# argmaxinc/WhisperKit

Hardware: AMD Instinct MI355X
Metric: audio-sec/sec (1/RTF), 30 s chunks: host PCM -> log-mel + encoder + greedy decode -> segments (higher is better)
Workload: dtype f16

## Files before the change

### whisperkit_amd/csrc/xabs.hip

```cpp
#include "dec_shared.h"
#include "knobs.h"

namespace wh {

typedef unsigned u32x4 __attribute__((ext_vector_type(4)));
typedef short s16x4 __attribute__((ext_vector_type(4)));
typedef f16 f16x2 __attribute__((ext_vector_type(2)));

__host__ __device__ __forceinline__ int xswz(int key) { return ((key & 3) << 2) | ((0x78 >> (2 * ((key >> 2) & 3))) & 3); }

__global__ void xabs_tile_wk_kernel(const f16* __restrict__ Wk, int d, int H, f16* __restrict__ out, size_t n_units) {
    const size_t o = (size_t)blockIdx.x * blockDim.x + threadIdx.x;
    if (o >= n_units) return;
    const int lane = (int)(o & 63);
    size_t t = o >> 6;
    const int kt = (int)(t & 3); t >>= 2;
    const int RT = d >> 5;
    const int rt = (int)(t % RT), h = (int)(t / RT);
    const int c = rt * 32 + (lane & 31), j0 = h * 64 + kt * 16 + 8 * (lane >> 5);
    f16x8 v;
#pragma unroll
    for (int i = 0; i < 8; ++i) v[i] = Wk[(size_t)(j0 + i) * d + c];
    *reinterpret_cast<f16x8*>(out + o * 8) = v;
}
void xabs_tile_wk(const f16* Wk, int d, int H, f16* out, hipStream_t st) {
    const size_t n_units = (size_t)H * (d / 32) * 4 * 64;
    xabs_tile_wk_kernel<<<(unsigned)((n_units + 255) / 256), 256, 0, st>>>(Wk, d, H, out, n_units);
}

template <int NHT, int WPB = 4>
__global__ __launch_bounds__(256, 2) void xabs_qk_kernel(const XabsArgs a) {
    const int tid = threadIdx.x, lane = tid & 63, wave = tid >> 6;
    const int h = blockIdx.y, bt = blockIdx.z;
    const int d = a.d, RT = d >> 5;
    const int j = lane & 31, hl = lane >> 5, gb = bt * 32 + j;
    f16x8 qh[4], ql[4];
    {
        const float* qp = a.q + (size_t)gb * d + h * 64 + hl * 8;
        float4 v0[4], v1[4];
#pragma unroll
        for (int kt = 0; kt < 4; ++kt) { v0[kt] = *reinterpret_cast<const float4*>(qp + kt * 16); v1[kt] = *reinterpret_cast<const float4*>(qp + kt * 16 + 4); }
#pragma unroll
        for (int kt = 0; kt < 4; ++kt) {
            const float z[8] = {v0[kt].x, v0[kt].y, v0[kt].z, v0[kt].w, v1[kt].x, v1[kt].y, v1[kt].z, v1[kt].w};
#pragma unroll
            for (int i = 0; i < 8; ++i) { f16 h_, l_; split_hilo(z[i], h_, l_); qh[kt][i] = h_; ql[kt][i] = l_; }
        }
    }
#pragma unroll
    for (int s = 0; s < 2; ++s) {
        const int rt = (blockIdx.x * WPB + wave) * 2 + s;
        const u32x4* wp = reinterpret_cast<const u32x4*>(a.wkT) + ((size_t)(h * RT + rt) * 4) * 64 + lane;
        u32x4 w[4];
#pragma unroll
        for (int kt = 0; kt < 4; ++kt) w[kt] = wp[kt * 64];
        f32x16 acc_h = {0}, acc_l = {0};
#pragma unroll
        for (int kt = 0; kt < 4; ++kt) {
            const f16x8 wf = __builtin_bit_cast(f16x8, w[kt]);
            acc_h = __builtin_amdgcn_mfma_f32_32x32x16_f16(wf, qh[kt], acc_h, 0, 0, 0);
            acc_l = __builtin_amdgcn_mfma_f32_32x32x16_f16(wf, ql[kt], acc_l, 0, 0, 0);
        }
        unsigned ph[4][2], pl[4][2];
#pragma unroll
        for (int g = 0; g < 4; ++g) {
            f16 zh[4], zl[4];
#pragma unroll
            for (int i = 0; i < 4; ++i) split_hilo(fmaf(acc_l[4 * g + i], 1.0f / 2048.0f, acc_h[4 * g + i]), zh[i], zl[i]);
            ph[g][0] = __builtin_bit_cast(unsigned, f16x2{zh[0], zh[1]});
            ph[g][1] = __builtin_bit_cast(unsigned, f16x2{zh[2], zh[3]});
            pl[g][0] = __builtin_bit_cast(unsigned, f16x2{zl[0], zl[1]});
            pl[g][1] = __builtin_bit_cast(unsigned, f16x2{zl[2], zl[3]});
        }
        u32x4 oh[2], ol[2];
#pragma unroll
        for (int u = 0; u < 2; ++u) {
#pragma unroll
            for (int i = 0; i < 2; ++i) {
                auto sh = __builtin_amdgcn_permlane32_swap(ph[u][i], ph[u + 2][i], false, false);
                auto sl = __builtin_amdgcn_permlane32_swap(pl[u][i], pl[u + 2][i], false, false);
                oh[u][i] = sh[0]; oh[u][2 + i] = sh[1];
                ol[u][i] = sl[0]; ol[u][2 + i] = sl[1];
            }
        }
        if (gb < a.batch) {
            const size_t o = ((size_t)gb * (NHT * 16) + h) * d + rt * 32 + 16 * hl;
            f16* lo_dst = h < 16 ? a.qf_lo + o : a.qf_hi + o + (size_t)8 * d;
#pragma unroll
            for (int u = 0; u < 2; ++u) {
                *reinterpret_cast<u32x4*>(a.qf_hi + o + 8 * u) = oh[u];
                *reinterpret_cast<u32x4*>(lo_dst + 8 * u) = ol[u];
            }
        }
    }
    if (a.gate && blockIdx.x == 0 && blockIdx.y == 0 && blockIdx.z == 0 && tid == 0) xattn_gate_acquire(a.gate);
}

template <int KSW, int NHT>
struct XabsQFrag { f16x8 h0[KSW], l0[KSW], p1[NHT == 2 ? KSW : 1]; };
template <int KSW, int NHT>
__device__ __forceinline__ void xabs_load_qfrag(const XabsArgs& a, int b, int c0, int lane, XabsQFrag<KSW, NHT>& q) {
    const int row = lane & 15, H = a.n_head, D = a.d;
    const size_t qo = ((size_t)b * (NHT * 16) + row) * D + c0 + (lane >> 4) * 8;
    const f16x8 zero = {0, 0, 0, 0, 0, 0, 0, 0};
    const bool real0 = row < H;
    const bool real1 = NHT == 2 && 16 + (row & 7) < H;
#pragma unroll
    for (int j = 0; j < KSW; ++j) {
        q.h0[j] = real0 ? *reinterpret_cast<const f16x8*>(a.qf_hi + qo + j * 32) : zero;
        q.l0[j] = real0 ? *reinterpret_cast<const f16x8*>(a.qf_lo + qo + j * 32) : zero;
        if constexpr (NHT == 2) q.p1[j] = real1 ? *reinterpret_cast<const f16x8*>(a.qf_hi + qo + (size_t)16 * D + j * 32) : zero;
    }
}
template <int KSW, int NHT>
__device__ __forceinline__ void xabs_s_tile(const f16x8 (&af)[KSW], const XabsQFrag<KSW, NHT>& q, int lane, float (&sreg)[NHT * 4]) {
    f32x4 sh = {0, 0, 0, 0}, sl = {0, 0, 0, 0}, sp = {0, 0, 0, 0};
#pragma unroll
    for (int j = 0; j < KSW; ++j) {
        sh = __builtin_amdgcn_mfma_f32_16x16x32_f16(af[j], q.h0[j], sh, 0, 0, 0);
        sl = __builtin_amdgcn_mfma_f32_16x16x32_f16(af[j], q.l0[j], sl, 0, 0, 0);
        if constexpr (NHT == 2) sp = __builtin_amdgcn_mfma_f32_16x16x32_f16(af[j], q.p1[j], sp, 0, 0, 0);
    }
#pragma unroll
    for (int r = 0; r < 4; ++r) sreg[r] = fmaf(sl[r], 1.0f / 2048.0f, sh[r]);
    if constexpr (NHT == 2) {
#pragma unroll
        for (int r = 0; r < 4; ++r) {
            const float lo = dpp_mov<kDppRor8>(sp[r]);
            sreg[4 + r] = (lane & 15) < 8 ? fmaf(lo, 1.0f / 2048.0f, sp[r]) : 0.0f;
        }
    }
}

constexpr int kXabsHalves = 7;
constexpr int kXabsSpStride = 32 * 17;
constexpr float kXabsDefer = 8.0f;
__host__ __device__ constexpr int xabs_lds_bytes_w(int nw, int ksw) { return kXabsHalves * 8 * nw * ksw * 64 + nw * kXabsSpStride * 4 + 1024 + 128; }
__host__ __device__ constexpr int xabs_lds_bytes(int cw) { return xabs_lds_bytes_w(8, cw); }

template <int KSW, int NHT, bool DBG, bool NTL, int NW = 8, bool MAP = false>
__global__ __launch_bounds__(NW * 64, 2) void xabs_attn_kernel(const XabsArgs a) {
    static_assert(NW == 8 || NW == 4, "the waves split the channels: 8, or 4 at d = 384");
    static_assert(4 * NW >= 16 * NHT, "4 softmax-owner heads per wave");
    constexpr int CW = KSW;
    constexpr int HWSH = NW == 8 ? 2 : 1, HW = NW / 2;
    constexpr int D = NW * KSW * 32, ROWB = D * 2, HALF = 8 * ROWB;
    static_assert(HALF == HW * CW * 1024, "a half tile is HW x CW pieces of 1 KB");
    extern __shared__ __attribute__((aligned(1024))) unsigned char smem[];
    float* spart = reinterpret_cast<float*>(smem + kXabsHalves * HALF);
    f16* pfrag = reinterpret_cast<f16*>(smem + kXabsHalves * HALF + NW * kXabsSpStride * 4);
    float* alpha_l = reinterpret_cast<float*>(smem + kXabsHalves * HALF + NW * kXabsSpStride * 4 + 1024);
    const int tid = threadIdx.x, lane = tid & 63;
    const int wave = __builtin_amdgcn_readfirstlane(tid >> 6);
    const int xr = blockIdx.x & 7, xq = blockIdx.x >> 3;
    const int S = a.n_split, H = a.n_head;
    const int spw = max(a.spw, 1), b1 = (a.batch + spw - 1) / spw;
    const int n_grp = (b1 + 3) >> 2, grp = (xq >> 2) * 8 + xr;
    const int sp = grp / n_grp, b_first = ((grp - sp * n_grp) << 2) + (xq & 3);
    if (a.gate && blockIdx.x == gridDim.x - 1 && tid == 0) xattn_gate_release(a.gate);
    if (sp >= S || b_first >= b1) return;
#define XPHASE(k) do { if constexpr (DBG) if (a.dbg && lane == 0 && (wave == 0 || wave == 5) && blockIdx.x < 64) \
        a.dbg[((blockIdx.x * 2 + (wave == 5)) * 2) * 16 + (k)] = __builtin_amdgcn_s_memtime(); } while (0)
    constexpr int NT = (kCtx + 15) / 16;
    const int tile_lo = sp * NT / S, tile_hi = (sp + 1) * NT / S, n = tile_hi - tile_lo;
  for (int b = b_first; b < a.batch; b += b1) {
    if (b != b_first) __syncthreads();
    XPHASE(9);
    int bc, bh = b;
    if constexpr (MAP) { bh = a.slot_home[b]; bc = bh; }
    else bc = a.cross_div > 1 ? b / a.cross_div : b;
    const unsigned char* enc = reinterpret_cast<const unsigned char*>(a.enc + (size_t)bc * kCtx * D);

    const int half_w = wave >> HWSH, wq = wave & (HW - 1);
    int p_off[CW];
#pragma unroll
    for (int p = 0; p < CW; ++p) {
        const int o = (wq * CW + p) * 1024 + lane * 16;
        const int row = o / ROWB, slot = (o - row * ROWB) >> 4;
        p_off[p] = (half_w * 8 + row) * ROWB + ((slot ^ xswz(half_w * 8 + row)) << 4);
    }
    int hi_mine = -1;
    auto issue = [&](int i) {
        unsigned char* dst = smem + ((2 * i + half_w) % kXabsHalves) * HALF + wq * (CW * 1024);
        const int t16 = (tile_lo + i) * 16;
#if defined(__HIP_DEVICE_COMPILE__)
        const __amdgpu_buffer_rsrc_t rs = __builtin_amdgcn_make_buffer_rsrc(const_cast<unsigned char*>(enc) + (size_t)t16 * ROWB, 0, (kCtx - t16) * ROWB, 0x00020000);
#pragma unroll
        for (int p = 0; p < CW; ++p)
            __builtin_amdgcn_raw_ptr_buffer_load_lds(rs, (__attribute__((address_space(3))) void*)(dst + p * 1024), 16, p_off[p], 0, 0, NTL ? 2 : 0);
#else
        (void)dst; (void)t16; (void)p_off;
#endif
        hi_mine = i;
    };
    auto wait_tile = [&](int k) {
        switch (hi_mine - k) {
            case 0: asm volatile("s_waitcnt vmcnt(0)" ::: "memory"); break;
            case 1: asm volatile("s_waitcnt vmcnt(%0)" ::"n"(CW) : "memory"); break;
            case 2: asm volatile("s_waitcnt vmcnt(%0)" ::"n"(2 * CW) : "memory"); break;
            default: asm volatile("s_waitcnt vmcnt(%0)" ::"n"(3 * CW) : "memory"); break;
        }
    };
    const SeqState* sq = a.seq + b;
    const int s_act = sq->active, s_done = sq->done, s_ti = sq->token_index;
    const int o_key = lane & 15, o_head = 4 * wave + (lane >> 4);
    const bool owner = o_head < 16 * NHT;
    int al_slot = -1;
    if (a.align && owner && o_head < H) al_slot = a.align_slot[a.layer * H + o_head];
    XabsQFrag<CW, NHT> qf;
    xabs_load_qfrag<CW, NHT>(a, b, wave * CW * 32, lane, qf);
    issue(0);
    if (n > 1) issue(1);
    if (n > 2) issue(2);
    if (n > 3 && half_w == 0) issue(3);
    if (tid < 32) alpha_l[tid] = 1.0f;
    if constexpr (NW == 8) pfrag[tid] = (f16)0.0f;
    else reinterpret_cast<unsigned*>(pfrag)[tid] = 0u;
    if (!(s_act && !s_done)) {
        asm volatile("s_waitcnt vmcnt(0)" ::: "memory");
        continue;
    }
    const int pos = min(max(s_ti, 0), kMaxTok - 1);
    float* raw = nullptr;
    if (al_slot >= 0 && pos + 1 < kMaxTok) raw = a.align + (((size_t)bh * kMaxTok + pos + 1) * a.n_align + al_slot) * kCtx;
    XPHASE(10);

    f32x16 acc[CW];
#pragma unroll
    for (int mt = 0; mt < CW; ++mt)
#pragma unroll
        for (int r = 0; r < 16; ++r) acc[mt][r] = 0.0f;
    float m_run = -INFINITY, l_run = 0.0f;
    const int s_key = lane & 15, s_kg = lane >> 4, s_sw = xswz(s_key);
    const int g16 = lane >> 4, sl = lane & 15;
    const int t_key0 = (g16 >> 1) * 8 + (sl >> 2), t_key1 = t_key0 + 4;
    const int t_c = (g16 & 1) * 2 + ((sl & 3) >> 1), t_b = (sl & 1) * 8;
    const int t_off0 = (t_key0 & 7) * ROWB + t_b, t_off1 = (t_key1 & 7) * ROWB + t_b, t_sw0 = xswz(t_key0), t_sw1 = xswz(t_key1);
    auto s_base = [&](int i) { return smem + ((2 * i + (s_key >> 3)) % kXabsHalves) * HALF + (s_key & 7) * ROWB; };
    auto t_base = [&](int i) { return smem + ((2 * i + (g16 >> 1)) % kXabsHalves) * HALF; };

    auto s_phase = [&](const unsigned char* row, float (&sreg)[NHT * 4]) {
        f16x8 af[CW];
#pragma unroll
        for (int j = 0; j < CW; ++j) {
            const int c = (wave * CW + j) * 4 + s_kg;
            af[j] = *reinterpret_cast<const f16x8*>(row + ((c ^ s_sw) << 4));
        }
        xabs_s_tile<CW, NHT>(af, qf, lane, sreg);
    };
    auto write_partials = [&](const float (&sreg)[NHT * 4]) {
        float* wpart = spart + wave * kXabsSpStride;
#pragma unroll
        for (int ht = 0; ht < NHT; ++ht)
#pragma unroll
            for (int r = 0; r < 4; ++r) wpart[(ht * 16 + (lane & 15)) * 17 + 4 * (lane >> 4) + r] = sreg[ht * 4 + r];
    };
    auto softmax = [&](int i) {
        float s = 0.0f;
#pragma unroll
        for (int v = 0; v < NW; ++v) s += spart[v * kXabsSpStride + o_head * 17 + o_key];
        const int t = (tile_lo + i) * 16 + o_key;
        const bool valid = t < kCtx;
        if (raw && valid) raw[t] = s;
        s = valid ? s : -INFINITY;
        float mt_ = s;
        mt_ = fmaxf(mt_, dpp_mov<kDppXor1>(mt_));
        mt_ = fmaxf(mt_, dpp_mov<kDppXor2>(mt_));
        mt_ = fmaxf(mt_, dpp_mov<kDppHalfMirror>(mt_));
        mt_ = fmaxf(mt_, dpp_mov<kDppMirror>(mt_));
        const float m_new = fmaxf(m_run, mt_);
        const float m_use = (m_new > m_run + kXabsDefer) ? m_new : m_run;
        const float al = __expf(m_run - m_use);
        float p = valid ? __expf(s - m_use) : 0.0f;
        if (o_head >= H) p = 0.0f;
        const f16 ph = (f16)p;
        float ps = (float)ph;
        ps += dpp_mov<kDppXor1>(ps);
        ps += dpp_mov<kDppXor2>(ps);
        ps += dpp_mov<kDppHalfMirror>(ps);
        ps += dpp_mov<kDppMirror>(ps);
        l_run = fmaf(l_run, al, ps);
        m_run = m_use;
        pfrag[(o_head | ((o_key >> 3) << 5)) * 8 + (o_key & 7)] = ph;
        if (o_key == 0) alpha_l[o_head] = (o_head < H) ? al : 1.0f;
    };
    auto pv = [&](const unsigned char* tile) {
        const f16x8 pf = *reinterpret_cast<const f16x8*>(pfrag + lane * 8);
        const float al = alpha_l[lane & 31];
        if (__builtin_amdgcn_ballot_w64(al != 1.0f)) {
#pragma unroll
            for (int mt = 0; mt < CW; ++mt)
#pragma unroll
                for (int r = 0; r < 16; ++r) acc[mt][r] *= al;
        }
#pragma unroll
        for (int mt = 0; mt < CW; ++mt) {
            const int c = (wave * CW + mt) * 4 + t_c;
            const s16x4 a0 = __builtin_amdgcn_ds_read_tr16_b64_v4i16((__attribute__((address_space(3))) s16x4*)(tile + t_off0 + ((c ^ t_sw0) << 4)));
            const s16x4 a1 = __builtin_amdgcn_ds_read_tr16_b64_v4i16((__attribute__((address_space(3))) s16x4*)(tile + t_off1 + ((c ^ t_sw1) << 4)));
            const f16x4 f0 = __builtin_bit_cast(f16x4, a0), f1 = __builtin_bit_cast(f16x4, a1);
            const f16x8 af = {f0[0], f0[1], f0[2], f0[3], f1[0], f1[1], f1[2], f1[3]};
            acc[mt] = __builtin_amdgcn_mfma_f32_32x32x16_f16(af, pf, acc[mt], 0, 0, 0);
        }
    };

    float sreg[NHT * 4];
    wait_tile(0);
    __syncthreads();
    s_phase(s_base(0), sreg);
    write_partials(sreg);
    if (n > 1) wait_tile(1);
    __syncthreads();
    XPHASE(11);
#define XSTAMP(k) do { if constexpr (DBG) if (a.dbg && (i == 10 || i == 11) && lane == 0 && (wave == 0 || wave == 5) && blockIdx.x < 64) \
        a.dbg[((blockIdx.x * 2 + (wave == 5)) * 2 + (i - 10)) * 16 + (k)] = __builtin_amdgcn_s_memtime(); } while (0)
    for (int i = 0; i < n; ++i) {
        XSTAMP(0);
        const bool work = !DBG || !(a.ablate & 2), fetch = !DBG || !(a.ablate & 1);
        if (work && i + 1 < n) s_phase(s_base(i + 1), sreg);
        XSTAMP(1);
        if (work && owner) softmax(i);
        XSTAMP(2);
        __syncthreads();
        XSTAMP(3);
        if (work && i + 1 < n) write_partials(sreg);
        XSTAMP(4);
        if (work) pv(t_base(i));
        XSTAMP(5);
        if (fetch && i + 2 < n) wait_tile(i + 2);
        XSTAMP(6);
        __syncthreads();
        XSTAMP(7);
        const int nx = i + 3 + (1 - half_w);
        if (fetch && nx < n) issue(nx);
        XSTAMP(8);
    }
#undef XSTAMP
    asm volatile("s_waitcnt vmcnt(0)" ::: "memory");
    XPHASE(12);
    if (owner && o_key == 0 && o_head < H) a.ml[((size_t)sp * H + o_head) * a.max_batch + b] = float2{m_run, l_run};
    {
        const int head = lane & 31, hl = lane >> 5;
        if (head < H) {
            float* pb = a.part + (((size_t)sp * H + head) * (D / 8)) * a.max_batch * 8 + (size_t)b * 8 + 4 * hl;
#pragma unroll
            for (int mt = 0; mt < CW; ++mt)
#pragma unroll
                for (int g = 0; g < 4; ++g) {
                    const int c8 = (wave * CW + mt) * 4 + g;
                    *reinterpret_cast<float4*>(pb + (size_t)c8 * a.max_batch * 8) = float4{acc[mt][4 * g], acc[mt][4 * g + 1], acc[mt][4 * g + 2], acc[mt][4 * g + 3]};
                }
        }
    }
    if constexpr (DBG) asm volatile("s_waitcnt vmcnt(0)" ::: "memory");
    XPHASE(13);
  }
#undef XPHASE
}


template <int S, int TW>
__global__ __launch_bounds__(256, 1) void xabs_vup_kernel(const XabsArgs a, int ks, int n_bt) {
    __shared__ float red[4][2][16][64];
    __shared__ int last_flag;
    const int tid = threadIdx.x, lane = tid & 63, wave = tid >> 6;
    const int d = a.d, H = a.n_head, KT = d >> 4;
    const int grp8 = blockIdx.x / (8 * n_bt), in8 = blockIdx.x % (8 * n_bt);
    const int xw = grp8 * 8 + (in8 & 7), bt = in8 >> 3;
    if (xw >= H * ks) return;
    const int h = xw % H, ksi = xw / H;
    const int kt0 = (ksi * 4 + wave) * TW;
    const int j = lane & 31, hl = lane >> 5;
    const int gbl = min(bt * 32 + j, a.max_batch - 1);
    float2 ml[S];
#pragma unroll
    for (int s = 0; s < S; ++s) ml[s] = a.ml[((size_t)s * H + h) * a.max_batch + gbl];
    const u32x4* wp = reinterpret_cast<const u32x4*>(a.wv_t) + ((size_t)(2 * h) * KT + kt0) * 64 + lane;
    const size_t sstride = (size_t)H * (d / 8) * a.max_batch * 8;
    const float* pp = a.part + ((size_t)h * (d / 8) + kt0 * 2 + hl) * a.max_batch * 8 + (size_t)gbl * 8;
    u32x4 w0[TW], w1[TW];
    f32x4 p0[TW][S], p1[TW][S];
#pragma unroll
    for (int i = 0; i < TW; ++i) { w0[i] = __builtin_nontemporal_load(wp + (size_t)i * 64); w1[i] = __builtin_nontemporal_load(wp + ((size_t)KT + i) * 64); }
#pragma unroll
    for (int i = 0; i < TW; ++i)
#pragma unroll
        for (int s = 0; s < S; ++s) {
            const float* q = pp + (size_t)s * sstride + (size_t)i * 2 * a.max_batch * 8;
            p0[i][s] = *reinterpret_cast<const f32x4*>(q);
            p1[i][s] = *reinterpret_cast<const f32x4*>(q + 4);
        }
#pragma unroll
    for (int i = 0; i < TW; ++i) {
        asm volatile("" : "+v"(w0[i]), "+v"(w1[i]));
#pragma unroll
        for (int s = 0; s < S; ++s) asm volatile("" : "+v"(p0[i][s]), "+v"(p1[i][s]));
    }
    float wn[S];
    {
        float mg = ml[0].x;
#pragma unroll
        for (int s = 1; s < S; ++s) mg = fmaxf(mg, ml[s].x);
        float lg = 0.0f;
#pragma unroll
        for (int s = 0; s < S; ++s) { wn[s] = __expf(ml[s].x - mg); lg = fmaf(wn[s], ml[s].y, lg); }
        const float inv = 1.0f / lg;
#pragma unroll
        for (int s = 0; s < S; ++s) wn[s] *= inv;
    }
    f32x16 acc_h[2] = {{0}, {0}}, acc_l[2] = {{0}, {0}};
#pragma unroll
    for (int i = 0; i < TW; ++i) {
        float z[8] = {0, 0, 0, 0, 0, 0, 0, 0};
#pragma unroll
        for (int s = 0; s < S; ++s) {
#pragma unroll
            for (int e = 0; e < 4; ++e) { z[e] = fmaf(wn[s], p0[i][s][e], z[e]); z[4 + e] = fmaf(wn[s], p1[i][s][e], z[4 + e]); }
        }
        f16x8 zh, zl;
#pragma unroll
        for (int e = 0; e < 8; ++e) { f16 h_, l_; split_hilo(z[e], h_, l_); zh[e] = h_; zl[e] = l_; }
        const f16x8 wf0 = __builtin_bit_cast(f16x8, w0[i]), wf1 = __builtin_bit_cast(f16x8, w1[i]);
        acc_h[0] = __builtin_amdgcn_mfma_f32_32x32x16_f16(wf0, zh, acc_h[0], 0, 0, 0);
        acc_l[0] = __builtin_amdgcn_mfma_f32_32x32x16_f16(wf0, zl, acc_l[0], 0, 0, 0);
        acc_h[1] = __builtin_amdgcn_mfma_f32_32x32x16_f16(wf1, zh, acc_h[1], 0, 0, 0);
        acc_l[1] = __builtin_amdgcn_mfma_f32_32x32x16_f16(wf1, zl, acc_l[1], 0, 0, 0);
    }
#pragma unroll
    for (int t = 0; t < 2; ++t)
#pragma unroll
        for (int r = 0; r < 16; ++r) red[wave][t][r][lane] = fmaf(acc_l[t][r], 1.0f / 2048.0f, acc_h[t][r]);
    __syncthreads();
    const int sub = tid >> 5, gb = bt * 32 + (tid & 31);
    float v[2][4];
#pragma unroll
    for (int t = 0; t < 2; ++t)
#pragma unroll
        for (int i = 0; i < 4; ++i) v[t][i] = ((red[0][t][4 * wave + i][lane] + red[1][t][4 * wave + i][lane]) + red[2][t][4 * wave + i][lane]) + red[3][t][4 * wave + i][lane];
    if (ks > 1) {
        float* base = a.kpart + (((size_t)bt * H + h) * ks) * 2048 + tid * 4;
#pragma unroll
        for (int t = 0; t < 2; ++t) {
            const f32x4 pv4 = {v[t][0], v[t][1], v[t][2], v[t][3]};
            float* mine = base + (size_t)ksi * 2048 + t * 1024;
            asm volatile("global_store_dwordx4 %0, %1, off sc1\n\ts_nop 1" ::"v"(mine), "v"(pv4) : "memory");
        }
        asm volatile("s_waitcnt vmcnt(0)" ::: "memory");
        __syncthreads();
        if (tid == 0) {
            int* cnt = a.ticket + bt * H + h;
            const int t = __hip_atomic_fetch_add(cnt, 1, __ATOMIC_RELAXED, __HIP_MEMORY_SCOPE_AGENT);
            const int last = (t == ks - 1);
            if (last) __hip_atomic_store(cnt, 0, __ATOMIC_RELAXED, __HIP_MEMORY_SCOPE_AGENT);
            last_flag = last;
        }
        __syncthreads();
        if (!last_flag) return;
        float pv[4][2][4];
#pragma unroll
        for (int s = 0; s < 4; ++s)
#pragma unroll
            for (int t = 0; t < 2; ++t) {
                const float* p = base + (size_t)(s < ks ? s : 0) * 2048 + t * 1024;
#pragma unroll
                for (int i = 0; i < 4; ++i) pv[s][t][i] = __hip_atomic_load(p + i, __ATOMIC_RELAXED, __HIP_MEMORY_SCOPE_AGENT);
            }
#pragma unroll
        for (int t = 0; t < 2; ++t)
#pragma unroll
            for (int i = 0; i < 4; ++i) {
                float x = pv[0][t][i];
#pragma unroll
                for (int s = 1; s < 4; ++s) x += (s < ks) ? pv[s][t][i] : 0.0f;
                v[t][i] = x;
            }
    }
    if (gb < a.batch && slot_live(a.seq + gb)) {
#pragma unroll
        for (int t = 0; t < 2; ++t) {
            const int nn = (2 * h + t) * 32 + 4 * sub;
            const float4 bv = *reinterpret_cast<const float4*>(a.bv + nn);
            const float y[4] = {v[t][0] + bv.x, v[t][1] + bv.y, v[t][2] + bv.z, v[t][3] + bv.w};
            f16x4 hi, lo;
#pragma unroll
            for (int i = 0; i < 4; ++i) { f16 h_, l_; split_hilo(y[i], h_, l_); hi[i] = h_; lo[i] = l_; }
            const size_t o = plane_index(gb, nn, d);
            *reinterpret_cast<f16x4*>(a.att_hi + o) = hi;
            *reinterpret_cast<f16x4*>(a.att_lo + o) = lo;
        }
    }
}

int xabs_splits(int max_batch) {
    const int e = knob::now<knob::WH_XABS_SPLITS>();
    return e ? e : xabs_auto_splits(max_batch);
}

void launch_xabs_qk(const XabsArgs& a, int n_bt, hipStream_t st) {
    ProfScope ps_(KK_DEC_XQK, st);
    if (a.d == 384) { xabs_qk_kernel<1, 2><<<dim3(3, a.n_head, n_bt), 128, 0, st>>>(a); return; }
    const dim3 grid(a.d / 256, a.n_head, n_bt);
    if (a.n_head > 16) xabs_qk_kernel<2><<<grid, 256, 0, st>>>(a);
    else xabs_qk_kernel<1><<<grid, 256, 0, st>>>(a);
}

template <int CW, int NHT, bool DBG, bool NTL, bool MAP = false>
static void launch_attn_k(const XabsArgs& a, hipStream_t st) {
    constexpr int lds = xabs_lds_bytes(CW);
    static PerDeviceOnce once;
    once.run([] { (void)hipFuncSetAttribute(reinterpret_cast<const void*>(&xabs_attn_kernel<CW, NHT, DBG, NTL, 8, MAP>), hipFuncAttributeMaxDynamicSharedMemorySize, lds); });
    xabs_attn_kernel<CW, NHT, DBG, NTL, 8, MAP><<<dim3(plan::xabs_attn_grid(a.batch, a.spw, a.n_split)), 512, lds, st>>>(a);
}
template <int KSW, bool DBG, bool NTL, bool MAP = false>
static void launch_attn_w4_k(const XabsArgs& a, hipStream_t st) {
    constexpr int lds = xabs_lds_bytes_w(4, KSW);
    static PerDeviceOnce once;
    once.run([] { (void)hipFuncSetAttribute(reinterpret_cast<const void*>(&xabs_attn_kernel<KSW, 1, DBG, NTL, 4, MAP>), hipFuncAttributeMaxDynamicSharedMemorySize, lds); });
    xabs_attn_kernel<KSW, 1, DBG, NTL, 4, MAP><<<dim3(plan::xabs_attn_grid(a.batch, a.spw, a.n_split)), 256, lds, st>>>(a);
}
template <int CW, int NHT, bool DBG, bool NTL, bool MAP = false>
static void launch_attn_any(const XabsArgs& a, hipStream_t st) {
    if constexpr (CW == 0) launch_attn_w4_k<3, DBG, NTL, MAP>(a, st); else launch_attn_k<CW, NHT, DBG, NTL, MAP>(a, st);
}
template <int CW, int NHT>
static void launch_attn_t(const XabsArgs& a, hipStream_t st) {
    const int nt = knob::once<knob::WH_XABS_NT>();
    const int ablate = knob::once<knob::WH_XABS_ABLATE>();
    if (a.mapped) { if (nt) launch_attn_any<CW, NHT, false, true, true>(a, st); else launch_attn_any<CW, NHT, false, false, true>(a, st); return; }
    if (a.dbg || ablate) { XabsArgs b = a; b.ablate = ablate; launch_attn_any<CW, NHT, true, false>(b, st); return; }
    if (nt && a.cross_div <= 1) launch_attn_any<CW, NHT, false, true>(a, st); else launch_attn_any<CW, NHT, false, false>(a, st);
}
void launch_xabs_attn(const XabsArgs& a, hipStream_t st) {
    ProfScope ps_(KK_DEC_CROSS_ATTN, st);
    const bool two = a.n_head > 16;
    switch (a.d / 256) {
        case 1: launch_attn_t<0, 1>(a, st); break;
        case 2: two ? launch_attn_t<2, 2>(a, st) : launch_attn_t<2, 1>(a, st); break;
        case 3: two ? launch_attn_t<3, 2>(a, st) : launch_attn_t<3, 1>(a, st); break;
        case 4: two ? launch_attn_t<4, 2>(a, st) : launch_attn_t<4, 1>(a, st); break;
        default: two ? launch_attn_t<5, 2>(a, st) : launch_attn_t<5, 1>(a, st); break;
    }
}

void launch_xabs_vup(const XabsArgs& a, int n_bt, hipStream_t st) {
    ProfScope ps_(KK_DEC_XVUP, st);
    const plan::XabsVupPlan p = plan::xabs_vup_plan(a.d, a.n_head, n_bt);
    const int ks = p.ks;
    const unsigned grid = p.grid;
#define XVUP(S_) do { switch (a.d / 256) { \
        case 1: xabs_vup_kernel<S_, 2><<<grid, 256, 0, st>>>(a, ks, n_bt); break; \
        case 2: xabs_vup_kernel<S_, 2><<<grid, 256, 0, st>>>(a, ks, n_bt); break; \
        case 3: xabs_vup_kernel<S_, 3><<<grid, 256, 0, st>>>(a, ks, n_bt); break; \
        case 4: xabs_vup_kernel<S_, 4><<<grid, 256, 0, st>>>(a, ks, n_bt); break; \
        default: xabs_vup_kernel<S_, 5><<<grid, 256, 0, st>>>(a, ks, n_bt); break; } } while (0)
    switch (a.n_split) {
        case 1: XVUP(1); break;
        case 2: XVUP(2); break;
        case 3: XVUP(3); break;
        default: XVUP(4); break;
    }
#undef XVUP
}

}
```

Before: 2629.

## Pipeline encoder tile prefetch across batch slots in cross-attention kernel

The cross-attention kernel now keeps one persistent tile ring across all live batch slots handled by a workgroup, instead of draining and restarting the prefetch pipeline for each slot. Slot liveness is gathered once with a wave ballot, so dead slots are skipped. The next slot's encoder tiles and query fragments are issued while the current slot is still being processed. The vmcnt waits are reworked to count the in-flight query loads and partial-result stores, and buffer loads to LDS are issued through inline asm with scalar descriptors. This removes pipeline bubbles between slots, at the cost of complex counter bookkeeping where a miscounted vmcnt threshold could cause data races.

```diff
diff --git a/whisperkit_amd/csrc/xabs.hip b/whisperkit_amd/csrc/xabs.hip
--- a/whisperkit_amd/csrc/xabs.hip
+++ b/whisperkit_amd/csrc/xabs.hip
@@ -1,5 +1,8 @@
+#include <type_traits>
+
 #include "dec_shared.h"
 #include "knobs.h"
+#include "xabs_ring.h"
 
 namespace wh {
 
@@ -132,7 +135,6 @@
     }
 }
 
-constexpr int kXabsHalves = 7;
 constexpr int kXabsSpStride = 32 * 17;
 constexpr float kXabsDefer = 8.0f;
 __host__ __device__ constexpr int xabs_lds_bytes_w(int nw, int ksw) { return kXabsHalves * 8 * nw * ksw * 64 + nw * kXabsSpStride * 4 + 1024 + 128; }
@@ -163,13 +165,29 @@
         a.dbg[((blockIdx.x * 2 + (wave == 5)) * 2) * 16 + (k)] = __builtin_amdgcn_s_memtime(); } while (0)
     constexpr int NT = (kCtx + 15) / 16;
     const int tile_lo = sp * NT / S, tile_hi = (sp + 1) * NT / S, n = tile_hi - tile_lo;
-  for (int b = b_first; b < a.batch; b += b1) {
-    if (b != b_first) __syncthreads();
+    static_assert(kXabsMaxSlotsPerWorkgroup <= 64, "one lane per slot of the workgroup's sequence");
     XPHASE(9);
-    int bc, bh = b;
-    if constexpr (MAP) { bh = a.slot_home[b]; bc = bh; }
-    else bc = a.cross_div > 1 ? b / a.cross_div : b;
-    const unsigned char* enc = reinterpret_cast<const unsigned char*>(a.enc + (size_t)bc * kCtx * D);
+    int l_ti = 0, l_home = 0;
+    bool l_live = false;
+    if (const int bl = b_first + lane * b1; bl < a.batch) {
+        const SeqState* sq = a.seq + bl;
+        const int s_act = sq->active, s_done = sq->done;
+        l_ti = sq->token_index;
+        l_live = (s_act != 0) & (s_done == 0);
+        if constexpr (MAP) l_home = a.slot_home[bl];
+    }
+    const unsigned long long live = __builtin_amdgcn_ballot_w64(l_live);
+    if (live == 0) return;
+    auto slot_of = [&](int k, int& b_, int& bh_) {
+        int bc;
+        b_ = b_first + k * b1; bh_ = b_;
+        if constexpr (MAP) { bh_ = __builtin_amdgcn_readlane(l_home, k); bc = bh_; }
+        else bc = a.cross_div > 1 ? b_ / a.cross_div : b_;
+        return reinterpret_cast<const unsigned char*>(a.enc + (size_t)bc * kCtx * D);
+    };
+    int ks = xring::next_live(live, -1), b, bh, g0 = 0;
+    const unsigned char* enc = slot_of(ks, b, bh);
+    const unsigned char* enc_nx = enc;
 
     const int half_w = wave >> HWSH, wq = wave & (HW - 1);
     int p_off[CW];
@@ -180,46 +198,68 @@
         p_off[p] = (half_w * 8 + row) * ROWB + ((slot ^ xswz(half_w * 8 + row)) << 4);
     }
     int hi_mine = -1;
-    auto issue = [&](int i) {
-        unsigned char* dst = smem + ((2 * i + half_w) % kXabsHalves) * HALF + wq * (CW * 1024);
-        const int t16 = (tile_lo + i) * 16;
+    int q_mark = -1, st_mark = -1;
+    auto issue = [&](int g) {
+        unsigned char* dst = smem + xring::ring_slot(g, half_w) * HALF + wq * (CW * 1024);
+        const bool cur = g < g0 + n;
+        const unsigned char* src = cur ? enc : enc_nx;
+        const int t16 = (tile_lo + (cur ? g - g0 : g - g0 - n)) * 16;
 #if defined(__HIP_DEVICE_COMPILE__)
-        const __amdgpu_buffer_rsrc_t rs = __builtin_amdgcn_make_buffer_rsrc(const_cast<unsigned char*>(enc) + (size_t)t16 * ROWB, 0, (kCtx - t16) * ROWB, 0x00020000);
-#pragma unroll
-        for (int p = 0; p < CW; ++p)
-            __builtin_amdgcn_raw_ptr_buffer_load_lds(rs, (__attribute__((address_space(3))) void*)(dst + p * 1024), 16, p_off[p], 0, 0, NTL ? 2 : 0);
+        const unsigned long long ba = reinterpret_cast<unsigned long long>(src) + (unsigned long long)t16 * ROWB;
+        const u32x4 rd = {(unsigned)__builtin_amdgcn_readfirstlane((int)(unsigned)ba), (unsigned)__builtin_amdgcn_readfirstlane((int)((unsigned)(ba >> 32) & 0xffffu)),
+                          (unsigned)__builtin_amdgcn_readfirstlane((kCtx - t16) * ROWB), 0x00020000u};
+        const unsigned m0v = (unsigned)__builtin_amdgcn_readfirstlane((int)((unsigned)(size_t)(__attribute__((address_space(3))) unsigned char*)smem + (unsigned)(dst - smem)));
+#pragma unroll
+        for (int p = 0; p < CW; ++p) {
+            if constexpr (NTL) asm volatile("s_mov_b32 m0, %2\n\ts_nop 0\n\tbuffer_load_dwordx4 %0, %1, 0 offen nt lds" ::"v"(p_off[p]), "s"(rd), "s"(m0v + p * 1024) : "memory");
+            else asm volatile("s_mov_b32 m0, %2\n\ts_nop 0\n\tbuffer_load_dwordx4 %0, %1, 0 offen lds" ::"v"(p_off[p]), "s"(rd), "s"(m0v + p * 1024) : "memory");
+        }
 #else
-        (void)dst; (void)t16; (void)p_off;
+        (void)dst; (void)src; (void)t16; (void)p_off;
 #endif
-        hi_mine = i;
-    };
-    auto wait_tile = [&](int k) {
-        switch (hi_mine - k) {
-            case 0: asm volatile("s_waitcnt vmcnt(0)" ::: "memory"); break;
-            case 1: asm volatile("s_waitcnt vmcnt(%0)" ::"n"(CW) : "memory"); break;
-            case 2: asm volatile("s_waitcnt vmcnt(%0)" ::"n"(2 * CW) : "memory"); break;
-            default: asm volatile("s_waitcnt vmcnt(%0)" ::"n"(3 * CW) : "memory"); break;
-        }
-    };
-    const SeqState* sq = a.seq + b;
-    const int s_act = sq->active, s_done = sq->done, s_ti = sq->token_index;
+        hi_mine = g;
+    };
+    constexpr int NQ = xring::q_loads(CW, NHT), NS = xring::part_stores(CW);
+    static_assert(xring::wait_threshold(0, 3, 0, 0, CW, NQ, NS) <= 63, "vmcnt has 6 bits");
+    auto wait_tile = [&](int g) {
+        const int t = min(hi_mine - g, 3);
+        if (g > max(q_mark, st_mark)) {
+            switch (t) {
+                case 0: asm volatile("s_waitcnt vmcnt(0)" ::: "memory"); break;
+                case 1: asm volatile("s_waitcnt vmcnt(%0)" ::"n"(CW) : "memory"); break;
+                case 2: asm volatile("s_waitcnt vmcnt(%0)" ::"n"(2 * CW) : "memory"); break;
+                default: asm volatile("s_waitcnt vmcnt(%0)" ::"n"(3 * CW) : "memory"); break;
+            }
+            return;
+        }
+#define XWAIT(T_, Q_, S_) case (T_) | (Q_) << 2 | (S_) << 3: \
+            asm volatile("s_waitcnt vmcnt(%0)" ::"n"(xring::wait_threshold(0, T_, (Q_) - 1, (S_) - 1, CW, NQ, NS)) : "memory"); break;
+        switch (t | (g <= q_mark ? 4 : 0) | (g <= st_mark ? 8 : 0)) {
+            XWAIT(0, 0, 0) XWAIT(1, 0, 0) XWAIT(2, 0, 0) XWAIT(3, 0, 0) XWAIT(0, 1, 0) XWAIT(1, 1, 0) XWAIT(2, 1, 0) XWAIT(3, 1, 0)
+            XWAIT(0, 0, 1) XWAIT(1, 0, 1) XWAIT(2, 0, 1) XWAIT(3, 0, 1) XWAIT(0, 1, 1) XWAIT(1, 1, 1) XWAIT(2, 1, 1) XWAIT(3, 1, 1)
+            default: asm volatile("s_waitcnt vmcnt(0)" ::: "memory"); break;
+        }
+#undef XWAIT
+    };
     const int o_key = lane & 15, o_head = 4 * wave + (lane >> 4);
     const bool owner = o_head < 16 * NHT;
     int al_slot = -1;
     if (a.align && owner && o_head < H) al_slot = a.align_slot[a.layer * H + o_head];
     XabsQFrag<CW, NHT> qf;
     xabs_load_qfrag<CW, NHT>(a, b, wave * CW * 32, lane, qf);
-    issue(0);
-    if (n > 1) issue(1);
-    if (n > 2) issue(2);
-    if (n > 3 && half_w == 0) issue(3);
+  for (;;) {
+    if (g0 != 0) {
+        __syncthreads();
+        XPHASE(9);
+    }
+    int kn = -1, bn = b, bhn = bh;
+    if (kn = xring::next_live(live, ks); kn >= 0) enc_nx = slot_of(kn, bn, bhn);
+    const bool follow = kn >= 0;
+    for (int g = hi_mine + 1; g < g0 + xring::prologue_goal(n, half_w); ++g) issue(g);
     if (tid < 32) alpha_l[tid] = 1.0f;
     if constexpr (NW == 8) pfrag[tid] = (f16)0.0f;
     else reinterpret_cast<unsigned*>(pfrag)[tid] = 0u;
-    if (!(s_act && !s_done)) {
-        asm volatile("s_waitcnt vmcnt(0)" ::: "memory");
-        continue;
-    }
+    const int s_ti = __builtin_amdgcn_readlane(l_ti, ks);
     const int pos = min(max(s_ti, 0), kMaxTok - 1);
     float* raw = nullptr;
     if (al_slot >= 0 && pos + 1 < kMaxTok) raw = a.align + (((size_t)bh * kMaxTok + pos + 1) * a.n_align + al_slot) * kCtx;
@@ -236,8 +276,8 @@
     const int t_key0 = (g16 >> 1) * 8 + (sl >> 2), t_key1 = t_key0 + 4;
     const int t_c = (g16 & 1) * 2 + ((sl & 3) >> 1), t_b = (sl & 1) * 8;
     const int t_off0 = (t_key0 & 7) * ROWB + t_b, t_off1 = (t_key1 & 7) * ROWB + t_b, t_sw0 = xswz(t_key0), t_sw1 = xswz(t_key1);
-    auto s_base = [&](int i) { return smem + ((2 * i + (s_key >> 3)) % kXabsHalves) * HALF + (s_key & 7) * ROWB; };
-    auto t_base = [&](int i) { return smem + ((2 * i + (g16 >> 1)) % kXabsHalves) * HALF; };
+    auto s_base = [&](int g) { return smem + xring::ring_slot(g, s_key >> 3) * HALF + (s_key & 7) * ROWB; };
+    auto t_base = [&](int g) { return smem + xring::ring_slot(g, g16 >> 1) * HALF; };
 
     auto s_phase = [&](const unsigned char* row, float (&sreg)[NHT * 4]) {
         f16x8 af[CW];
@@ -304,20 +344,32 @@
         }
     };
 
+    auto load_next_q = [&]() {
+        if (!follow) return;
+        asm volatile("" ::: "memory");
+        xabs_load_qfrag<CW, NHT>(a, bn, wave * CW * 32, lane, qf);
+        q_mark = hi_mine;
+        asm volatile("" ::: "memory");
+    };
     float sreg[NHT * 4];
-    wait_tile(0);
+    wait_tile(g0);
     __syncthreads();
-    s_phase(s_base(0), sreg);
+    s_phase(s_base(g0), sreg);
     write_partials(sreg);
-    if (n > 1) wait_tile(1);
+    if (n == 1) load_next_q();
+    if (n > 1) wait_tile(g0 + 1);
     __syncthreads();
     XPHASE(11);
 #define XSTAMP(k) do { if constexpr (DBG) if (a.dbg && (i == 10 || i == 11) && lane == 0 && (wave == 0 || wave == 5) && blockIdx.x < 64) \
         a.dbg[((blockIdx.x * 2 + (wave == 5)) * 2 + (i - 10)) * 16 + (k)] = __builtin_amdgcn_s_memtime(); } while (0)
-    for (int i = 0; i < n; ++i) {
+    using WithQ = std::true_type;
+    using NoQ = std::false_type;
+    auto tile_step = [&](const int i, auto lq) __attribute__((always_inline)) {
+        const int g = g0 + i;
         XSTAMP(0);
         const bool work = !DBG || !(a.ablate & 2), fetch = !DBG || !(a.ablate & 1);
-        if (work && i + 1 < n) s_phase(s_base(i + 1), sreg);
+        if (work && i + 1 < n) s_phase(s_base(g + 1), sreg);
+        if constexpr (decltype(lq)::value) load_next_q();
         XSTAMP(1);
         if (work && owner) softmax(i);
         XSTAMP(2);
@@ -325,18 +377,21 @@
         XSTAMP(3);
         if (work && i + 1 < n) write_partials(sreg);
         XSTAMP(4);
-        if (work) pv(t_base(i));
+        if (work) pv(t_base(g));
         XSTAMP(5);
-        if (fetch && i + 2 < n) wait_tile(i + 2);
+        if (fetch && i + 2 < n) wait_tile(g + 2);
         XSTAMP(6);
         __syncthreads();
         XSTAMP(7);
-        const int nx = i + 3 + (1 - half_w);
-        if (fetch && nx < n) issue(nx);
+        if (fetch) { if (const int nx = xring::loop_request(g0, n, i, half_w, hi_mine, follow); nx >= 0) issue(nx); }
         XSTAMP(8);
-    }
+    };
+    for (int i = 0; i < n - 2; ++i) tile_step(i, NoQ{});
+    if (n >= 2) tile_step(n - 2, WithQ{});
+    tile_step(n - 1, NoQ{});
 #undef XSTAMP
-    asm volatile("s_waitcnt vmcnt(0)" ::: "memory");
+    if (!follow) asm volatile("s_waitcnt vmcnt(0)" ::: "memory");
+    else asm volatile("" ::: "memory");
     XPHASE(12);
     if (owner && o_key == 0 && o_head < H) a.ml[((size_t)sp * H + o_head) * a.max_batch + b] = float2{m_run, l_run};
     {
@@ -352,8 +407,11 @@
                 }
         }
     }
+    st_mark = hi_mine;
     if constexpr (DBG) asm volatile("s_waitcnt vmcnt(0)" ::: "memory");
     XPHASE(13);
+    if (!follow) break;
+    ks = kn; b = bn; bh = bhn; enc = enc_nx; g0 += n;
   }
 #undef XPHASE
 }
diff --git a/whisperkit_amd/csrc/xabs_ring.h b/whisperkit_amd/csrc/xabs_ring.h
--- /dev/null
+++ b/whisperkit_amd/csrc/xabs_ring.h
@@ -0,0 +1,34 @@
+#pragma once
+
+#if defined(__HIPCC__)
+#define XRING_HD __host__ __device__
+#else
+#define XRING_HD
+#endif
+
+namespace wh {
+
+constexpr int kXabsHalves = 7;
+
+namespace xring {
+
+XRING_HD constexpr int next_live(unsigned long long live, int k) {
+    const unsigned long long rest = k >= 63 ? 0ull : live >> (k + 1);
+    return rest ? k + 1 + __builtin_ctzll(rest) : -1;
+}
+XRING_HD constexpr int ring_slot(int g, int half) { return (2 * g + half) % kXabsHalves; }
+XRING_HD constexpr int lead(int half_w) { return 3 + (1 - half_w); }
+XRING_HD constexpr int prologue_goal(int n, int half_w) { return n < lead(half_w) ? n : lead(half_w); }
+XRING_HD constexpr int loop_request(int g0, int n, int i, int half_w, int hi, bool follow) {
+    const int t = hi + 1, limit = g0 + i + lead(half_w), end = g0 + n + (follow ? n : 0);
+    return (t <= limit && t < end) ? t : -1;
+}
+XRING_HD constexpr int q_loads(int ksw, int nht) { return (2 + (nht == 2 ? 1 : 0)) * ksw; }
+XRING_HD constexpr int part_stores(int ksw) { return 4 * ksw; }
+XRING_HD constexpr int wait_threshold(int k, int hi, int q_mark, int st_mark, int ksw, int nq, int ns) {
+    const int t = hi - k < 3 ? hi - k : 3;
+    return t * ksw + (k <= q_mark ? nq : 0) + (k <= st_mark ? ns : 0);
+}
+
+}
+}
```

New measurement: 2630, median of 2. Within noise of the previous version (+0.0%).
